# AiRyunn/BoT

Measured on NVIDIA B200. Metric: GAT layer fwd+bwd edges/sec (ogbn-proteins shape), higher is better.
Workload: dtype f32

## Files before the change

bot_b200/csrc/edge_ops.cu:

```cuda
#include "common.cuh"

namespace botgat {

static int env_pf() {
  const char* s = getenv("BOTGAT_PF");
  return (s && *s) ? atoi(s) : 0;
}

template <int PF> __device__ __forceinline__ float4 ld_rec4(const float* p) {
  float4 r;
  if constexpr (PF == 64)
    asm("ld.global.nc.L2::64B.v4.f32 {%0,%1,%2,%3}, [%4];" : "=f"(r.x), "=f"(r.y), "=f"(r.z), "=f"(r.w) : "l"(p));
  else if constexpr (PF == 128)
    asm("ld.global.nc.L2::128B.v4.f32 {%0,%1,%2,%3}, [%4];" : "=f"(r.x), "=f"(r.y), "=f"(r.z), "=f"(r.w) : "l"(p));
  else if constexpr (PF == 256)
    asm("ld.global.nc.L2::256B.v4.f32 {%0,%1,%2,%3}, [%4];" : "=f"(r.x), "=f"(r.y), "=f"(r.z), "=f"(r.w) : "l"(p));
  else
    r = __ldg(reinterpret_cast<const float4*>(p));
  return r;
}
template <int PF> __device__ __forceinline__ float2 ld_rec2(const float* p) {
  float2 r;
  if constexpr (PF == 64) asm("ld.global.nc.L2::64B.v2.f32 {%0,%1}, [%2];" : "=f"(r.x), "=f"(r.y) : "l"(p));
  else if constexpr (PF == 128) asm("ld.global.nc.L2::128B.v2.f32 {%0,%1}, [%2];" : "=f"(r.x), "=f"(r.y) : "l"(p));
  else if constexpr (PF == 256) asm("ld.global.nc.L2::256B.v2.f32 {%0,%1}, [%2];" : "=f"(r.x), "=f"(r.y) : "l"(p));
  else r = __ldg(reinterpret_cast<const float2*>(p));
  return r;
}
template <int PF> __device__ __forceinline__ float ld_rec1(const float* p) {
  float r;
  if constexpr (PF == 64) asm("ld.global.nc.L2::64B.f32 %0, [%1];" : "=f"(r) : "l"(p));
  else if constexpr (PF == 128) asm("ld.global.nc.L2::128B.f32 %0, [%1];" : "=f"(r) : "l"(p));
  else if constexpr (PF == 256) asm("ld.global.nc.L2::256B.f32 %0, [%1];" : "=f"(r) : "l"(p));
  else r = __ldg(p);
  return r;
}

constexpr int kHMax = 8;

template <int VEC, int PF> __device__ __forceinline__ void load_record(const float* rec, int H, float (&v)[kHMax]) {
  if constexpr (VEC == 4) {
#pragma unroll
    for (int q = 0; q < kHMax / 4; ++q) {
      if (q * 4 < H) {
        const float4 t = ld_rec4<PF>(rec + q * 4);
        v[q * 4] = t.x; v[q * 4 + 1] = t.y; v[q * 4 + 2] = t.z; v[q * 4 + 3] = t.w;
      }
    }
  } else if constexpr (VEC == 2) {
#pragma unroll
    for (int q = 0; q < kHMax / 2; ++q) {
      if (q * 2 < H) {
        const float2 t = ld_rec2<PF>(rec + q * 2);
        v[q * 2] = t.x; v[q * 2 + 1] = t.y;
      }
    }
  } else {
#pragma unroll
    for (int q = 0; q < kHMax; ++q)
      if (q < H) v[q] = ld_rec1<PF>(rec + q);
  }
}
template <int VEC> __device__ __forceinline__ void store_record(float* rec, int H, const float (&v)[kHMax]) {
  if constexpr (VEC == 4) {
#pragma unroll
    for (int q = 0; q < kHMax / 4; ++q)
      if (q * 4 < H) *reinterpret_cast<float4*>(rec + q * 4) = make_float4(v[q * 4], v[q * 4 + 1], v[q * 4 + 2], v[q * 4 + 3]);
  } else if constexpr (VEC == 2) {
#pragma unroll
    for (int q = 0; q < kHMax / 2; ++q)
      if (q * 2 < H) *reinterpret_cast<float2*>(rec + q * 2) = make_float2(v[q * 2], v[q * 2 + 1]);
  } else {
#pragma unroll
    for (int q = 0; q < kHMax; ++q)
      if (q < H) rec[q] = v[q];
  }
}

static int record_vec(const void* p, int64_t ld, int H) {
  auto fits = [&](int w) { return ld % w == 0 && ((uintptr_t)p % (4 * w)) == 0 && ((H + w - 1) / w) * w <= ld; };
  return fits(4) ? 4 : (fits(2) ? 2 : 1);
}

__global__ void k_pack_keep(int64_t n_edges, const uint8_t* __restrict__ keep, uint32_t* __restrict__ bits) {
  const int64_t n_round = (n_edges + 31) & ~(int64_t)31;
  for (int64_t e = blockIdx.x * (int64_t)blockDim.x + threadIdx.x; e < n_round; e += (int64_t)gridDim.x * blockDim.x) {
    const unsigned b = __ballot_sync(0xffffffffu, e < n_edges && __ldg(keep + e) != 0);
    if ((threadIdx.x & 31) == 0) bits[e >> 5] = b;
  }
}

template <int VEC, int PF>
__global__ void k_edge_stage(int64_t n_edges, int h0, int Hn, const int32_t* __restrict__ eid,
                             const int32_t* __restrict__ order,
                             const float* __restrict__ src, int64_t ld, const uint8_t* __restrict__ keep,
                             const uint32_t* __restrict__ keep_bits, float* __restrict__ dst) {
  for (int64_t t = blockIdx.x * (int64_t)blockDim.x + threadIdx.x; t < n_edges; t += (int64_t)gridDim.x * blockDim.x) {
    const int64_t p = order ? __ldg(order + t) : t;
    const int64_t e = __ldg(eid + p);
    float v[kHMax];
#pragma unroll
    for (int q = 0; q < kHMax; ++q) v[q] = 0.f;
    if (src) load_record<VEC, PF>(src + e * ld + h0, Hn, v);
    const bool dropped = keep_bits ? !((__ldg(keep_bits + (e >> 5)) >> (e & 31)) & 1u) : (keep && !__ldg(keep + e));
#pragma unroll
    for (int q = 0; q < kHMax; ++q)
      if (q < Hn) dst[(int64_t)(h0 + q) * n_edges + p] = dropped ? -INFINITY : v[q];
  }
}

template <int VEC>
__global__ void k_edge_unstage(int64_t n_edges, int h0, int Hn, int Hw, const int32_t* __restrict__ eid,
                               const int32_t* __restrict__ order,
                               const float* __restrict__ gz, float* __restrict__ dst, int64_t ld) {
  for (int64_t t = blockIdx.x * (int64_t)blockDim.x + threadIdx.x; t < n_edges; t += (int64_t)gridDim.x * blockDim.x) {
    const int64_t p = order ? __ldg(order + t) : t;
    const int64_t e = __ldg(eid + p);
    float v[kHMax];
#pragma unroll
    for (int q = 0; q < kHMax; ++q) v[q] = (q < Hn) ? __ldg(gz + (int64_t)(h0 + q) * n_edges + p) : 0.f;
    store_record<VEC>(dst + e * ld + h0, Hw, v);
  }
}

template <int VEC, int PF>
__global__ void __launch_bounds__(256)
k_edge_reduce_dst(int n_items, int H, int h0, int Hn, const int32_t* __restrict__ indptr, const int32_t* __restrict__ eid,
                  const int32_t* __restrict__ seg_row, const int32_t* __restrict__ seg_beg,
                  const int32_t* __restrict__ seg_end, const int32_t* __restrict__ seg_slot,
                  const float* __restrict__ grad_ee, int64_t ld, float* __restrict__ grad_er, float* __restrict__ scratch) {
  const int warp = threadIdx.x >> 5, lane = threadIdx.x & 31;
  const int item = blockIdx.x * 8 + warp;
  if (item >= n_items) return;
  const int v = seg_row ? seg_row[item] : item;
  const int beg = seg_row ? seg_beg[item] : indptr[v], end = seg_row ? seg_end[item] : indptr[v + 1];
  const int slot = seg_row ? seg_slot[item] : -1;
  float s[kHMax];
#pragma unroll
  for (int q = 0; q < kHMax; ++q) s[q] = 0.f;
  for (int pos = beg + lane; pos < end; pos += 32) {
    float r[kHMax];
#pragma unroll
    for (int q = 0; q < kHMax; ++q) r[q] = 0.f;
    load_record<VEC, PF>(grad_ee + (int64_t)__ldg(eid + pos) * ld + h0, Hn, r);
#pragma unroll
    for (int q = 0; q < kHMax; ++q) s[q] += r[q];
  }
#pragma unroll
  for (int q = 0; q < kHMax; ++q) {
    if (q < Hn) {
      const float t = warp_sum(s[q]);
      if (lane == 0) {
        if (slot >= 0) scratch[(int64_t)slot * H + h0 + q] = t;
        else grad_er[(int64_t)v * H + h0 + q] = t;
      }
    }
  }
}

__global__ void k_edge_reduce_combine(int n_split, int H, const int32_t* __restrict__ split_rows,
                                      const int32_t* __restrict__ split_first, const float* __restrict__ scratch,
                                      float* __restrict__ grad_er) {
  const int t = blockIdx.x * blockDim.x + threadIdx.x;
  if (t >= n_split * H) return;
  const int i = t / H, h = t - i * H;
  float a = 0.f;
  for (int s = split_first[i]; s < split_first[i + 1]; ++s) a += scratch[(int64_t)s * H + h];
  grad_er[(int64_t)split_rows[i] * H + h] = a;
}

static inline int grid_for(int64_t n, int block = 256) {
  int64_t b = (n + block - 1) / block;
  return (int)std::max<int64_t>(1, std::min<int64_t>(b, 148 * 32));
}

#define BG_PF_SWITCH(CALL)                        \
  switch (pf) {                                   \
    case 64: { constexpr int PF = 64; CALL; break; }   \
    case 128: { constexpr int PF = 128; CALL; break; } \
    case 256: { constexpr int PF = 256; CALL; break; } \
    default: { constexpr int PF = 0; CALL; break; }    \
  }

static int stage_one(const botgat_graph* g, const int32_t* eid, const int32_t* order, int H, const float* src, int64_t ld,
                     const uint8_t* keep, float* dst, cudaStream_t st) {
  const int pf = env_pf();
  uint32_t* keep_bits = nullptr;
  const bool coalesced = eid == g->in_eid && g->in_eid_identity;
  if (keep && src && g->n_edges >= (1 << 20) && !coalesced) {
    BG_CHECK(cudaMallocAsync(&keep_bits, sizeof(uint32_t) * (size_t)((g->n_edges + 31) / 32), st));
    k_pack_keep<<<grid_for(g->n_edges), 256, 0, st>>>(g->n_edges, keep, keep_bits);
    BG_LAUNCHED(1);
  }
  struct FreeBits {
    uint32_t* p; cudaStream_t st;
    ~FreeBits() { if (p) cudaFreeAsync(p, st); }
  } free_bits{keep_bits, st};
  for (int h0 = 0; h0 < H; h0 += kHMax) {
    const int Hn = std::min(kHMax, H - h0);
    const int vec = src ? record_vec(src + h0, ld, Hn) : 1;
    const int grid = order ? (int)((g->n_edges + 255) / 256) : grid_for(g->n_edges);
    if (vec == 4) { BG_PF_SWITCH((k_edge_stage<4, PF><<<grid, 256, 0, st>>>(g->n_edges, h0, Hn, eid, order, src, ld, keep, keep_bits, dst))) }
    else if (vec == 2) { BG_PF_SWITCH((k_edge_stage<2, PF><<<grid, 256, 0, st>>>(g->n_edges, h0, Hn, eid, order, src, ld, keep, keep_bits, dst))) }
    else { BG_PF_SWITCH((k_edge_stage<1, PF><<<grid, 256, 0, st>>>(g->n_edges, h0, Hn, eid, order, src, ld, keep, keep_bits, dst))) }
    BG_LAUNCHED(1);
    BG_CHECK(cudaGetLastError());
  }
  return 0;
}

}

using namespace botgat;

extern "C" int botgat_edge_stage(const botgat_graph* g, int order, int32_t H, const float* ee, int64_t ld_ee,
                                 const uint8_t* keep, const float* attn_mul, int64_t ld_am, float* eb, float* am,
                                 void* stream) {
  BG_REQUIRE(g && H > 0, "edge_stage: bad arguments");
  BG_REQUIRE(order == BOTGAT_ORDER_IN || order == BOTGAT_ORDER_OUT, "edge_stage: bad order %d", order);
  BG_REQUIRE((eb != nullptr) == (ee != nullptr || keep != nullptr), "edge_stage: eb must be given iff ee or keep is");
  BG_REQUIRE((am != nullptr) == (attn_mul != nullptr), "edge_stage: am must be given iff attn_mul is");
  BG_REQUIRE(!ee || ld_ee >= H, "edge_stage: ld_ee < H");
  BG_REQUIRE(!attn_mul || ld_am >= H, "edge_stage: ld_am < H");
  if (g->n_edges == 0 || (!eb && !am)) return 0;
  DeviceGuard guard(g->device);
  cudaStream_t st = (cudaStream_t)stream;
  const int32_t* eid = order == BOTGAT_ORDER_IN ? g->in_eid : g->out_eid;
  const int32_t* visit = order == BOTGAT_ORDER_OUT ? g->out_tile_order : nullptr;
  if (eb) {
    int rc = stage_one(g, eid, visit, ee ? H : 1, ee, ld_ee, keep, eb, st);
    if (rc) return rc;
  }
  if (am) {
    int rc = stage_one(g, eid, visit, H, attn_mul, ld_am, nullptr, am, st);
    if (rc) return rc;
  }
  return 0;
}

extern "C" int botgat_edge_unstage(const botgat_graph* g, int order, int32_t H, const float* gz, float* grad_ee,
                                   int64_t ld_gee, void* stream) {
  BG_REQUIRE(g && H > 0, "edge_unstage: bad arguments");
  BG_REQUIRE(order == BOTGAT_ORDER_IN || order == BOTGAT_ORDER_OUT, "edge_unstage: bad order %d", order);
  if (g->n_edges == 0) return 0;
  BG_REQUIRE(gz && grad_ee, "edge_unstage: null gz/grad_ee");
  BG_REQUIRE(ld_gee >= H, "edge_unstage: ld_gee < H");
  DeviceGuard guard(g->device);
  cudaStream_t st = (cudaStream_t)stream;
  const int32_t* eid = order == BOTGAT_ORDER_IN ? g->in_eid : g->out_eid;
  const int32_t* visit = order == BOTGAT_ORDER_OUT ? g->out_tile_order : nullptr;
  for (int h0 = 0; h0 < ld_gee; h0 += kHMax) {
    const int Hn = std::max(0, std::min(kHMax, H - h0));
    const int Hw = (int)std::min<int64_t>(kHMax, ld_gee - h0);
    const int vec = record_vec(grad_ee + h0, ld_gee, Hw);
    const int grid = visit ? (int)((g->n_edges + 255) / 256) : grid_for(g->n_edges);
    if (vec == 4) k_edge_unstage<4><<<grid, 256, 0, st>>>(g->n_edges, h0, Hn, Hw, eid, visit, gz, grad_ee, ld_gee);
    else if (vec == 2) k_edge_unstage<2><<<grid, 256, 0, st>>>(g->n_edges, h0, Hn, Hw, eid, visit, gz, grad_ee, ld_gee);
    else k_edge_unstage<1><<<grid, 256, 0, st>>>(g->n_edges, h0, Hn, Hw, eid, visit, gz, grad_ee, ld_gee);
    BG_LAUNCHED(1);
    BG_CHECK(cudaGetLastError());
  }
  return 0;
}

extern "C" int botgat_edge_reduce_dst(const botgat_graph* g, int32_t H, const float* grad_ee, int64_t ld_gee,
                                      float* grad_er, float* scratch, void* stream) {
  BG_REQUIRE(g && H > 0 && grad_er, "edge_reduce_dst: bad arguments");
  BG_REQUIRE(grad_ee || g->n_edges == 0, "edge_reduce_dst: null grad_ee");
  BG_REQUIRE(ld_gee >= H || g->n_edges == 0, "edge_reduce_dst: ld_gee < H");
  if (g->n_dst == 0) return 0;
  DeviceGuard guard(g->device);
  cudaStream_t st = (cudaStream_t)stream;
  const int pf = env_pf();
  const botgat_graph::SegTable& seg = g->seg_in;
  const bool split = seg.n_items > 0;
  BG_REQUIRE(!split || seg.n_slots == 0 || scratch, "edge_reduce_dst: this graph has split rows; scratch (n_slots_in*H floats) is required");
  const int n_items = split ? seg.n_items : (int)g->n_dst;
  const int32_t *sr = split ? seg.row : nullptr, *sb = seg.beg, *se = seg.end, *ss = seg.slot;
  const int grid = (n_items + 7) / 8;
  for (int h0 = 0; h0 < H; h0 += kHMax) {
    const int Hn = std::min(kHMax, H - h0);
    const int vec = g->n_edges ? record_vec(grad_ee + h0, ld_gee, Hn) : 1;
#define BG_RD(VEC) BG_PF_SWITCH((k_edge_reduce_dst<VEC, PF><<<grid, 256, 0, st>>>(n_items, H, h0, Hn, g->in_indptr, g->in_eid, sr, sb, se, ss, grad_ee, ld_gee, grad_er, scratch)))
    if (vec == 4) { BG_RD(4) } else if (vec == 2) { BG_RD(2) } else { BG_RD(1) }
#undef BG_RD
    BG_LAUNCHED(1);
    BG_CHECK(cudaGetLastError());
  }
  if (split && seg.n_split > 0) {
    const int n = seg.n_split * H;
    k_edge_reduce_combine<<<(n + 255) / 256, 256, 0, st>>>(seg.n_split, H, seg.split_rows, seg.split_first, scratch, grad_er);
    BG_LAUNCHED(1);
    BG_CHECK(cudaGetLastError());
  }
  return 0;
}
```

bot_b200/functional.py:

```python
from __future__ import annotations

import ctypes as C
import os

import torch

from . import _lib
from .graph import Graph, _stream


class KernelTimer:

    def __init__(self):
        self.events = []

    def span(self, name):
        return _Span(self, name)

    def totals(self):
        out = {}
        for name, s, e in self.events:
            n, t = out.get(name, (0, 0.0))
            out[name] = (n + 1, t + s.elapsed_time(e))
        return out


class _Span:
    def __init__(self, timer, name):
        self.timer, self.name = timer, name

    def __enter__(self):
        if self.timer is not None:
            self.s = torch.cuda.Event(enable_timing=True)
            self.s.record()

    def __exit__(self, *exc):
        if self.timer is not None:
            e = torch.cuda.Event(enable_timing=True)
            e.record()
            self.timer.events.append((self.name, self.s, e))


timer = None

edge_mode = "staged"

prestage_backward = False
_side_streams = {}


def _side_stream(device):
    key = (device.type, device.index)
    if key not in _side_streams:
        _side_streams[key] = torch.cuda.Stream(device=device)
    return _side_streams[key]


def _span(name):
    return _Span(timer, name)


def _r4(x):
    return (x + 3) // 4 * 4


def _f32c(t, name):
    if t is None:
        return None
    if t.dtype != torch.float32:
        raise TypeError(f"{name}: expected float32, got {t.dtype}")
    if not t.is_cuda:
        raise RuntimeError(f"{name}: bot_b200 has no CPU path — tensor must be on a CUDA device")
    return t.contiguous()


def _rows(t, name, H):
    if t is None:
        return None, 0
    if t.dtype != torch.float32 or not t.is_cuda:
        raise TypeError(f"{name}: expected a float32 CUDA tensor")
    if t.dim() != 2 or t.shape[1] < H:
        raise ValueError(f"{name}: expected (E, >= {H}), got {tuple(t.shape)}")
    if t.stride(1) != 1 or t.stride(0) < t.shape[1]:
        t = t.contiguous()
    return t, t.stride(0)


def pad_heads(H):
# ... 15 lines not shown
        am = torch.empty((H, E), dtype=torch.float32, device=dev)
    if eb is None and am is None:
        return None, 0, None
    ee, ld_ee = _rows(ee, "ee", H)
    attn_mul, ld_am = _rows(attn_mul, "attn_mul", H)
    with _span("edge_stage"):
        rc = _lib.load().botgat_edge_stage(graph._ensure(), order, H, _lib.ptr(ee), ld_ee, _lib.ptr(keep),
                                           _lib.ptr(attn_mul), ld_am, _lib.ptr(eb), _lib.ptr(am), _stream())
    _lib.check(rc, "botgat_edge_stage")
    return eb, Hb, am


def _check_edge_operands(graph, H, ee, keep, attn_mul):
    E = graph.number_of_edges()
    ee, ld_ee = _rows(ee, "ee", H)
    attn_mul, ld_am = _rows(attn_mul, "attn_mul", H)
    if ee is not None and ee.shape[0] != E:
        raise ValueError("ee must have one row per edge")
    if keep is not None:
        keep = keep.to(torch.uint8).contiguous()
        if keep.numel() != E:
            raise ValueError("keep must have one entry per edge")
    return ee, ld_ee, keep, attn_mul, ld_am


def _forward_core(graph, ft2d, H, D, el, er, ee, ld_ee, keep, attn_mul, ld_am, src_scale, dst_scale, slope, attn_p, seed,
                  hooks, will_backward, ep=None):
    lib = _lib.load()
    h = graph._ensure()
    dev = ft2d.device
    N_d = graph.number_of_dst_nodes()
    staged = edge_mode == "staged"
    eb_in, Hb, am_in = edge_stage(graph, _lib.ORDER_IN, H, ee, keep, attn_mul) if staged else (None, 0, None)
    pre = None
    has_edge_ops = ee is not None or keep is not None or attn_mul is not None
    if staged and prestage_backward and has_edge_ops and will_backward:
        main, side = torch.cuda.current_stream(), _side_stream(dev)
        side.wait_stream(main)
        with torch.cuda.stream(side):
            eb_o, _, am_o = edge_stage(graph, _lib.ORDER_OUT, H, ee, keep, attn_mul)
            ev = torch.cuda.Event()
            ev.record(side)
        for t in (ee, keep, attn_mul):
            if t is not None:
                t.record_stream(side)
        pre = (eb_o, am_o, ev)
    out = torch.empty((N_d, H, D), dtype=torch.float32, device=dev)
    row_max = torch.empty((N_d, H), dtype=torch.float32, device=dev)
    row_sum = torch.empty((N_d, H), dtype=torch.float32, device=dev)
    a = _lib.FwdArgs()
    a.H, a.D, a.ld_ft, a.ld_out = H, D, ft2d.stride(0), H * D
    a.ft, a.el, a.er = ft2d.data_ptr(), el.data_ptr(), (er.data_ptr() if er is not None else None)
    a.eb, a.Hb, a.col_parts = (eb_in.data_ptr() if eb_in is not None else None), Hb, 0
    a.am = am_in.data_ptr() if am_in is not None else None
    if not staged:
        if (ee is not None and ld_ee != H) or (attn_mul is not None and ld_am != H):
            raise ValueError("direct edge mode needs unpadded (E,H) edge operands")
        a.ee = ee.data_ptr() if ee is not None else None
        a.keep = keep.data_ptr() if keep is not None else None
        a.attn_mul = attn_mul.data_ptr() if attn_mul is not None else None
    a.src_scale = src_scale.data_ptr() if src_scale is not None else None
    a.dst_scale = dst_scale.data_ptr() if dst_scale is not None else None
    a.slope, a.attn_p, a.seed = float(slope), float(attn_p if attn_mul is None else 0.0), int(seed)
    a.out, a.row_max, a.row_sum = out.data_ptr(), row_max.data_ptr(), row_sum.data_ptr()
    if ep is not None:
        if will_backward:
            raise RuntimeError("the fused layer epilogue is forward-only (the backward expects the plain aggregate)")
        for key, ld in (("res", "ld_res"), ("res2", "ld_res2")):
            t = ep.get(key)
            if t is not None:
                if t.dim() != 2 or t.shape[0] < N_d or t.shape[1] < H * D or t.stride(1) != 1 or t.dtype != torch.float32:
                    raise ValueError(f"epilogue {key} must be a float32 (>= N_dst, >= H*D) matrix with unit column stride")
                setattr(a, key, t.data_ptr())
                setattr(a, ld, t.stride(0))
        if ep.get("want_y", True):
            y = torch.empty((N_d, H * D), dtype=torch.float32, device=dev)
            ep["y"] = y
            a.y, a.ld_y = y.data_ptr(), H * D
            for key, field in (("scale", "ep_scale"), ("shift", "ep_shift")):
                t = ep.get(key)
                if t is not None:
                    t = ep[key] = _f32c(t, key)
                    if t.numel() != H * D:
                        raise ValueError(f"epilogue {key} must have H*D entries")
                    setattr(a, field, t.data_ptr())
            a.ep_relu = 1 if ep.get("relu") else 0
    scratch = None
    if graph._info.n_slots_in:
        scratch = torch.empty(graph._info.n_slots_in * _r4(H * (D + 2)), dtype=torch.float32, device=dev)
        a.scratch = scratch.data_ptr()
    if hooks is not None and hooks.pre_kernel is not None:
        hooks.pre_kernel()
    chunks = hooks.head_chunks if hooks is not None and hooks.head_chunks else [(0, H)]
    for i, (hb, hc) in enumerate(chunks):
        if len(chunks) > 1 and hooks.pre_head is not None:
            hooks.pre_head(i)
        a.h_begin, a.h_count = hb, hc
        with _span("gat_fwd"):
            rc = lib.botgat_gat_forward(h, C.byref(a), _stream())
        _lib.check(rc, "botgat_gat_forward")
    return out, row_max, row_sum, pre, float(a.attn_p)


def _backward_core(graph, cfg, pre, hooks, ft2d, el, er, ee, keep, attn_mul, src_scale, dst_scale, out, row_max, row_sum,
                   gout, grad_ft2d, need_er, need_ee, hook_grad_ft=None):
    lib = _lib.load()
    h = graph._ensure()
    H, D, staged, slope, attn_p, seed = cfg
    N_s, N_d, E = ft2d.shape[0], out.shape[0], graph.number_of_edges()
    dev = ft2d.device

    def p(t):
        return t.data_ptr() if t is not None else None

    if pre is not None:
        eb_out, am_out, ev = pre
        cur = torch.cuda.current_stream()
        cur.wait_event(ev)
        for t in (eb_out, am_out):
            if t is not None:
                t.record_stream(cur)
        Hb = eb_out.shape[0] if eb_out is not None else 0
    else:
        eb_out, Hb, am_out = edge_stage(graph, _lib.ORDER_OUT, H, ee, keep, attn_mul) if staged else (None, 0, None)
    drec = torch.empty((H, N_d, 4), dtype=torch.float32, device=dev)
    gprime = torch.empty_like(gout) if dst_scale is not None else None
    grad_el = torch.empty((N_s, H), dtype=torch.float32, device=dev)
    grad_er = torch.empty((N_d, H), dtype=torch.float32, device=dev) if need_er else None
    gz = grad_ee = None
    if need_er or need_ee:
        gz = torch.empty((H, E), dtype=torch.float32, device=dev) if staged else None
        Hp = ee.shape[1] if (ee is not None and staged) else (pad_heads(H) if staged else H)
        grad_ee = torch.empty((E, Hp), dtype=torch.float32, device=dev)
    a = _lib.BwdArgs()
    a.H, a.D, a.ld_ft, a.ld_out, a.ld_gft = H, D, ft2d.stride(0), H * D, grad_ft2d.stride(0)
    a.ft, a.el, a.er = ft2d.data_ptr(), el.data_ptr(), p(er)
    a.eb_out, a.Hb, a.phases, a.am_out = p(eb_out), Hb, 0, p(am_out)
    if not staged:
        a.ee, a.keep, a.attn_mul = p(ee), p(keep), p(attn_mul)
    a.src_scale, a.dst_scale = p(src_scale), p(dst_scale)
    a.slope, a.attn_p, a.seed = slope, attn_p, seed
    a.out, a.row_max, a.row_sum, a.gout = out.data_ptr(), row_max.data_ptr(), row_sum.data_ptr(), gout.data_ptr()
    a.drec, a.gprime, a.gz = drec.data_ptr(), p(gprime), p(gz)
    scratch = None
    if graph._info.n_slots_out or graph._info.n_slots_in:
        scratch = torch.empty(graph._info.n_slots_out * _r4(H * (D + 1)) + graph._info.n_slots_in * H,
                              dtype=torch.float32, device=dev)
        a.scratch = scratch.data_ptr()
    a.grad_ft, a.grad_el, a.grad_ee, a.grad_er = grad_ft2d.data_ptr(), grad_el.data_ptr(), p(grad_ee), p(grad_er)
    a.ld_gee = grad_ee.stride(0) if grad_ee is not None else 0
    post_src = hooks.post_src if hooks is not None else None
    chunks = hooks.head_chunks if hooks is not None and hooks.head_chunks else None
    if chunks is not None and (len(chunks) > 1 or getattr(hooks, "force_chunked", False)):
        a.phases = 1
        _lib.check(lib.botgat_gat_backward(h, C.byref(a), _stream()), "botgat_gat_backward")
        for i, (hb, hc) in enumerate(chunks):
            a.phases, a.h_begin, a.h_count = 2, hb, hc
# ... 25 lines not shown
    return grad_el, grad_er, (grad_ee if need_ee else None)


BWD_MAX_D = 1024


class GATFusedFn(torch.autograd.Function):

    @staticmethod
    def forward(ctx, graph, ft, el, er, ee, keep, attn_mul, src_scale, dst_scale, slope, attn_p, seed, hooks=None):
        if ft.dim() != 3:
            raise ValueError("ft must be (N_src, H, D)")
        ft = _f32c(ft, "ft")
        N_s, H, D = ft.shape
        N_d = graph.number_of_dst_nodes()
        if N_s != graph.number_of_src_nodes():
            raise ValueError(f"ft has {N_s} rows, graph has {graph.number_of_src_nodes()} source nodes")
        el = _f32c(el, "el").view(N_s, H)
        er = None if er is None else _f32c(er, "er").view(N_d, H)
        ee, ld_ee, keep, attn_mul, ld_am = _check_edge_operands(graph, H, ee, keep, attn_mul)
        src_scale, dst_scale = _f32c(src_scale, "src_scale"), _f32c(dst_scale, "dst_scale")
        Dk = D
        if any(ctx.needs_input_grad):
            if D > BWD_MAX_D:
                raise ValueError(f"GAT layer with gradients: head width D={D} exceeds the backward's limit of {BWD_MAX_D} "
                                 "columns per head (inference without gradients has no such limit)")
            vw = 4 if D % 4 == 0 and ft.data_ptr() % 16 == 0 else 2 if D % 2 == 0 and ft.data_ptr() % 8 == 0 else 1
            if D > 256 * vw:
                if hooks is not None:
                    raise ValueError(f"GAT layer with hooks: D={D} > {256 * vw} needs a multiple of 4 and a 16-byte aligned ft")
                Dk = _r4(D)
                ft = torch.cat([ft, ft.new_zeros(N_s, H, Dk - D)], 2)
        with torch.cuda.device(ft.device):
            out, row_max, row_sum, pre, attn_p_used = _forward_core(
                graph, ft.view(N_s, H * Dk), H, Dk, el, er, ee, ld_ee, keep, attn_mul, ld_am, src_scale, dst_scale, slope,
                attn_p, seed, hooks, any(ctx.needs_input_grad))
        ctx.graph = graph
        ctx.hooks = hooks
        ctx.pre = pre
        ctx.D = D
        ctx.cfg = (H, Dk, edge_mode == "staged", float(slope), attn_p_used, int(seed))
        ctx.save_for_backward(ft, el, er, ee, keep, attn_mul, src_scale, dst_scale, out, row_max, row_sum)
        return out if Dk == D else out[:, :, :D].contiguous()

    @staticmethod
    def backward(ctx, gout):
        ft, el, er, ee, keep, attn_mul, src_scale, dst_scale, out, row_max, row_sum = ctx.saved_tensors
        H, D = ctx.cfg[0], ctx.cfg[1]
        need_er = er is not None and ctx.needs_input_grad[3]
        need_ee = ee is not None and ctx.needs_input_grad[4]
        gout = _f32c(gout, "grad_out")
        if D != ctx.D:
            gout = torch.cat([gout, gout.new_zeros(gout.shape[0], H, D - ctx.D)], 2)
        elif D > 256 and gout.data_ptr() % 16:
            gout = gout.clone()
        grad_ft = torch.empty_like(ft)
        with torch.cuda.device(ft.device):
            grad_el, grad_er, grad_ee = _backward_core(
                ctx.graph, ctx.cfg, ctx.pre, ctx.hooks, ft.view(-1, H * D), el, er, ee, keep, attn_mul, src_scale, dst_scale,
                out, row_max, row_sum, gout, grad_ft.view(-1, H * D), need_er, need_ee, hook_grad_ft=grad_ft)
        if D != ctx.D:
            grad_ft = grad_ft[:, :, :ctx.D]
        return (None, grad_ft, grad_el, grad_er, grad_ee, None, None, None, None, None, None, None, None)


def _pad_rows(w, rows):
    if w.shape[0] == rows:
        return w
    return torch.cat([w, w.new_zeros(rows - w.shape[0], w.shape[1])], 0)


class GATConvSampledFn(torch.autograd.Function):

    @staticmethod
    def forward(ctx, graph, x_src, x_dst, w_src, w_dst, b_dst, ee, keep, attn_mul, dst_scale, H, D, slope, attn_p, seed,
                src_scale=None):
        x_src, x_dst = _f32c(x_src, "feat_src"), _f32c(x_dst, "feat_dst")
        N_s, N_d, HD = graph.number_of_src_nodes(), graph.number_of_dst_nodes(), H * D
        if x_src.shape[0] != N_s or x_dst.shape[0] != N_d:
            raise ValueError("feat_src / feat_dst rows do not match the graph")
        has_er = w_dst.shape[0] == HD + H
        P = (HD + H + 31) // 32 * 32
        ws, wd = _pad_rows(w_src, P), _pad_rows(w_dst, P)
        bd = torch.cat([b_dst, b_dst.new_zeros(P - HD)])
        ee, ld_ee, keep, attn_mul, ld_am = _check_edge_operands(graph, H, ee, keep, attn_mul)
        dst_scale, src_scale = _f32c(dst_scale, "dst_scale"), _f32c(src_scale, "src_scale")
        vw = 4 if D % 4 == 0 else 2 if D % 2 == 0 else 1
        if any(ctx.needs_input_grad) and D > min(256 * vw, BWD_MAX_D):
            raise ValueError(f"GAT layer with gradients: head width D={D} exceeds the backward's limit of {256 * vw} columns "
                             f"per head at {vw}-float vectors (at most {BWD_MAX_D}, for D a multiple of 4)")
        with torch.cuda.device(x_src.device):
            Ys = x_src @ ws.t()
            Yd = torch.addmm(bd, x_dst, wd.t())
            el = Ys[:, HD:HD + H].contiguous() if src_scale is None else Ys[:, HD:HD + H] * src_scale.unsqueeze(-1)
            er = Yd[:, HD:HD + H].contiguous() if has_er else None
            out, row_max, row_sum, pre, attn_p_used = _forward_core(
                graph, Ys, H, D, el, er, ee, ld_ee, keep, attn_mul, ld_am, src_scale, dst_scale, slope, attn_p, seed, None,
                any(ctx.needs_input_grad))
            rst = out + Yd[:, :HD].view(N_d, H, D)
        ctx.graph, ctx.pre, ctx.same_x = graph, pre, x_dst is x_src or x_dst.data_ptr() == x_src.data_ptr() and N_s == N_d
        ctx.cfg = (H, D, edge_mode == "staged", float(slope), attn_p_used, int(seed))
        ctx.dims = (P, has_er, w_src.shape[0], w_dst.shape[0])
        ctx.save_for_backward(x_src, x_dst, ws, wd, Ys, el, er, ee, keep, attn_mul, dst_scale, out, row_max, row_sum, src_scale)
        return rst

    @staticmethod
    def backward(ctx, grst):
        x_src, x_dst, ws, wd, Ys, el, er, ee, keep, attn_mul, dst_scale, out, row_max, row_sum, src_scale = ctx.saved_tensors
        H, D = ctx.cfg[0], ctx.cfg[1]
        P, has_er, rows_s, rows_d = ctx.dims
        HD = H * D
        need = ctx.needs_input_grad
        need_ee = ee is not None and need[6]
        grst = _f32c(grst, "grad_out")
        N_s, N_d = x_src.shape[0], x_dst.shape[0]
        dev = x_src.device
        with torch.cuda.device(dev):
            gYs = torch.empty((N_s, P), dtype=torch.float32, device=dev)
            gYd = torch.empty((N_d, P), dtype=torch.float32, device=dev)
            grad_el, grad_er, grad_ee = _backward_core(
                ctx.graph, ctx.cfg, ctx.pre, None, Ys, el, er, ee, keep, attn_mul, src_scale, dst_scale, out, row_max, row_sum,
                grst, gYs, has_er, need_ee)
            gYs[:, HD:HD + H] = grad_el if src_scale is None else grad_el * src_scale.unsqueeze(-1)
            gYs[:, HD + H:].zero_()
            gYd[:, :HD] = grst.view(N_d, HD)
            if has_er:
                gYd[:, HD:HD + H] = grad_er
                gYd[:, HD + H:].zero_()
            else:
                gYd[:, HD:].zero_()
            gw_s = (gYs.t() @ x_src)[:rows_s] if need[3] else None
            gw_d = (gYd.t() @ x_dst)[:rows_d] if need[4] else None
            gb = grst.view(N_d, HD).sum(0) if need[5] else None
            gx_s = gx_d = None
            if ctx.same_x and need[1]:
                gx_s = torch.addmm(gYs @ ws, gYd, wd)
            else:
                gx_s = gYs @ ws if need[1] else None
                gx_d = gYd @ wd if need[2] else None
        return (None, gx_s, gx_d, gw_s, gw_d, gb, grad_ee, None, None, None, None, None, None, None, None, None)


class LayerTail:

    def __init__(self, h_last=None, norm=None, relu=False):
        self.h_last, self.norm, self.relu = h_last, norm, relu

    def usable(self):
        if os.environ.get("BOTGAT_FUSE_TAIL", "1") == "0":
            return False
        n = self.norm
        if isinstance(n, torch.nn.BatchNorm1d):
            return not n.training and n.running_mean is not None
        return n is None or (hasattr(n, "weight") and hasattr(n, "bias"))

    def scale_shift(self):
        n = self.norm
        if n is None:
            return None, None
        if isinstance(n, torch.nn.BatchNorm1d):
            scale = torch.rsqrt(n.running_var + n.eps)
            if n.weight is not None:
                scale = scale * n.weight
            shift = -n.running_mean * scale
            if n.bias is not None:
                shift = shift + n.bias
            return scale.detach(), shift.detach()
        return (None if n.weight is None else n.weight.detach()), (None if n.bias is None else n.bias.detach())


def gat_fused_inference(graph, ft, el, er, ee, keep, attn_mul, src_scale, dst_scale, slope, tail, res=None):
    with torch.no_grad():
        ft = _f32c(ft, "ft")
        N_s, H, D = ft.shape
        N_d = graph.number_of_dst_nodes()
        el = _f32c(el, "el").view(N_s, H)
        er = None if er is None else _f32c(er, "er").view(N_d, H)
        ee, ld_ee, keep, attn_mul, ld_am = _check_edge_operands(graph, H, ee, keep, attn_mul)
        src_scale, dst_scale = _f32c(src_scale, "src_scale"), _f32c(dst_scale, "dst_scale")
        scale, shift = tail.scale_shift()
        h_last = tail.h_last
        if h_last is not None:
            h_last = _f32c(h_last, "h_last").view(h_last.shape[0], -1)
        if res is not None:
            res = _f32c(res, "res").view(res.shape[0], -1)
        ep = {"res": res, "res2": h_last, "scale": scale, "shift": shift, "relu": tail.relu, "want_y": True}
        with torch.cuda.device(ft.device):
            out, _, _, _, _ = _forward_core(graph, ft.view(N_s, H * D), H, D, el, er, ee, ld_ee, keep, attn_mul, ld_am, src_scale,
                                            dst_scale, slope, 0.0, 0, None, False, ep=ep)
        return out.view(N_d, H * D), ep["y"]


def gat_conv_inference(graph, x_src, x_dst, w_src, w_dst, b_dst, ee, keep, attn_mul, dst_scale, H, D, slope, tail,
                       src_scale=None):
    with torch.no_grad():
        x_src, x_dst = _f32c(x_src, "feat_src"), _f32c(x_dst, "feat_dst")
        N_s, N_d, HD = graph.number_of_src_nodes(), graph.number_of_dst_nodes(), H * D
        if x_src.shape[0] != N_s or x_dst.shape[0] != N_d:
            raise ValueError("feat_src / feat_dst rows do not match the graph")
        has_er = w_dst.shape[0] == HD + H
        P = (HD + H + 31) // 32 * 32
        ws, wd = _pad_rows(w_src, P), _pad_rows(w_dst, P)
        bd = torch.cat([b_dst, b_dst.new_zeros(P - HD)])
        ee, ld_ee, keep, attn_mul, ld_am = _check_edge_operands(graph, H, ee, keep, attn_mul)
        dst_scale, src_scale = _f32c(dst_scale, "dst_scale"), _f32c(src_scale, "src_scale")
        scale, shift = tail.scale_shift()
        h_last = tail.h_last
        if h_last is not None:
            h_last = _f32c(h_last, "h_last").view(h_last.shape[0], -1)
        ep = {"res2": h_last, "scale": scale, "shift": shift, "relu": tail.relu, "want_y": True}
        with torch.cuda.device(x_src.device):
            Ys = x_src @ ws.t()
            Yd = torch.addmm(bd, x_dst, wd.t())
            ep["res"] = Yd
            el = Ys[:, HD:HD + H].contiguous() if src_scale is None else Ys[:, HD:HD + H] * src_scale.unsqueeze(-1)
            er = Yd[:, HD:HD + H].contiguous() if has_er else None
            out, _, _, _, _ = _forward_core(graph, Ys, H, D, el, er, ee, ld_ee, keep, attn_mul, ld_am, src_scale, dst_scale,
                                            slope, 0.0, 0, None, False, ep=ep)
        return out.view(N_d, HD), ep["y"]


class EdgeLogitProj(torch.autograd.Function):

    @staticmethod
    def forward(ctx, x, weight):
        lib = _lib.load()
        x = _f32c(x, "feat_edge")
        weight = _f32c(weight, "weight")
        E, Cin = x.shape
        H = weight.shape[0]
        y = torch.empty((E, pad_heads(H)), dtype=torch.float32, device=x.device)
        with torch.cuda.device(x.device):
            with _span("edge_proj_fwd"):
                rc = lib.botgat_edge_proj_forward(E, Cin, H, x.data_ptr(), x.stride(0), weight.data_ptr(), y.data_ptr(),
                                                  y.stride(0), x.device.index, _stream())
        _lib.check(rc, "botgat_edge_proj_forward")
        ctx.save_for_backward(x, weight)
        return y

    @staticmethod
    def backward(ctx, gy):
        lib = _lib.load()
        x, weight = ctx.saved_tensors
        E, Cin = x.shape
        H = weight.shape[0]
        gy, ld_gy = _rows(gy, "grad_ee", H)
        gx = torch.empty_like(x) if ctx.needs_input_grad[0] else None
        gw = torch.empty_like(weight) if ctx.needs_input_grad[1] else None
        partials = torch.empty(lib.botgat_edge_proj_gw_blocks() * H * Cin, dtype=torch.float32, device=x.device) \
            if gw is not None else None
# ... 144 lines not shown
```

bot_b200/partition.py:

```python
from __future__ import annotations

import os

import torch
import torch.distributed as dist

from .graph import Graph


def partition_bounds(dst, n_nodes, n_parts):
    counts = torch.bincount(dst, minlength=n_nodes)
    indptr = torch.zeros(n_nodes + 1, dtype=torch.int64, device=dst.device)
    indptr[1:] = torch.cumsum(counts, 0)
    e = int(dst.numel())
    targets = torch.tensor([(p * e) // n_parts for p in range(1, n_parts)], dtype=torch.int64, device=dst.device)
    inner = torch.searchsorted(indptr, targets, right=False).clamp(max=n_nodes)
    bounds = torch.cat([torch.zeros(1, dtype=torch.int64, device=dst.device), inner,
                        torch.full((1,), n_nodes, dtype=torch.int64, device=dst.device)])
    return torch.cummax(bounds, 0).values


class _DenseHalo(torch.autograd.Function):

    @staticmethod
# ... 149 lines not shown
        n_own = pg.n_own
        graph = pg.local
        main = torch.cuda.current_stream()
        if hx.fwd_pending:
            hx.h_table.barrier(channel=0)
        hx.fwd_pending, hx.bwd_pending = True, False
        if ft_own.data_ptr() != hx.own_ft.data_ptr():
            hx.own[:, :HD].copy_(ft_own.reshape(n_own, HD))
        if el_own.data_ptr() != hx.own_el.data_ptr():
            hx.own_el.copy_(el_own.reshape(n_own, H))
        hx.h_table.barrier(channel=1)
        hx.stream.wait_stream(main)
        events = []
        with torch.cuda.stream(hx.stream):
            for i, (hb, hc) in enumerate(chunks):
                if i == 0:
                    hx.pull(HD, H)
                hx.pull(hb * D, hc * D)
                ev = torch.cuda.Event()
                ev.record(hx.stream)
                events.append(ev)
        el_all = torch.empty((hx.table.shape[0], H), dtype=torch.float32, device=hx.table.device)

        def pre_kernel():
            main.wait_event(events[0])
            el_all.copy_(hx.table[:, HD:HD + H])

        def pre_head(i):
            if i > 0:
                main.wait_event(events[i])

        ee, ld_ee, keep, attn_mul, ld_am = Fn._check_edge_operands(graph, H, ee, keep, attn_mul)
        hooks = Fn.Hooks(pre_kernel=pre_kernel, head_chunks=chunks, pre_head=pre_head)
        out, row_max, row_sum, pre, attn_p_used = Fn._forward_core(
            graph, hx.table, H, D, el_all, er, ee, ld_ee, keep, attn_mul, ld_am, src_scale, dst_scale, slope, attn_p, seed,
            hooks, True)
        ctx.pg, ctx.hx, ctx.chunks = pg, hx, chunks
        ctx.cfg = (H, D, Fn.edge_mode == "staged", float(slope), attn_p_used, int(seed))
        ctx.save_for_backward(el_all, er, ee, keep, attn_mul, src_scale, dst_scale, out, row_max, row_sum)
        return out

    @staticmethod
    def backward(ctx, gout):
        from . import functional as Fn

        pg, hx, chunks = ctx.pg, ctx.hx, ctx.chunks
        el_all, er, ee, keep, attn_mul, src_scale, dst_scale, out, row_max, row_sum = ctx.saved_tensors
        H, D, HD = hx.H, hx.D, hx.HD
        n_own = pg.n_own
        main = torch.cuda.current_stream()
        gout = gout.contiguous()
        gshard = torch.empty((hx.rows, hx.P), dtype=torch.float32, device=gout.device)
        gshard.record_stream(hx.stream)
        if hx.bwd_pending or not hx.fwd_pending:
            hx.h_gtable.barrier(channel=0)
        hx.bwd_pending, hx.fwd_pending = True, False

        def post_src_head(i, grad_ft, grad_el):
            hb, hc = chunks[i]
            last = i == len(chunks) - 1
            if last:
                hx.gtable[:, HD:HD + H].copy_(grad_el)
            ev = torch.cuda.Event()
            ev.record(main)
            with torch.cuda.stream(hx.stream):
                hx.stream.wait_event(ev)
                hx.h_gtable.barrier(channel=1 + i)
                hx.pull_reduce(hb * D, hc * D, gshard)
                if last:
                    hx.pull_reduce(HD, H, gshard)

        hooks = Fn.Hooks(head_chunks=chunks, post_src_head=post_src_head)
        hooks.force_chunked = True
        need_er = er is not None and ctx.needs_input_grad[5]
        need_ee = ee is not None and ctx.needs_input_grad[6]
        grad_el, grad_er, grad_ee = Fn._backward_core(
            pg.local, ctx.cfg, None, hooks, hx.table, el_all, er, ee, keep, attn_mul, src_scale, dst_scale, out, row_max, row_sum,
            gout, hx.gtable, need_er, need_ee)
        main.wait_stream(hx.stream)
        grad_ft_own = gshard[:n_own, :HD].unflatten(1, (H, D))
        grad_el_own = gshard[:n_own, HD:HD + H]
        return (None, None, None, grad_ft_own, grad_el_own, grad_er, grad_ee, None, None, None, None, None, None, None)


class PartitionedGraph:

    def __init__(self, src, dst, n_nodes, world=None, rank=None, group=None, plan="auto", build_graph=True):
        self.group = group
        self.pipeline_heads = os.environ.get("BOTGAT_PIPE_HEADS", "0") == "1"
        self.exchange = os.environ.get("BOTGAT_EXCHANGE", "auto")
        self.halo_chunks = int(os.environ.get("BOTGAT_HALO_CHUNKS", "0"))
        self._p2p, self._p2p_failed, self._p2p_error = {}, False, None
        self.world = dist.get_world_size(group) if world is None else world
        self.rank = dist.get_rank(group) if rank is None else rank
        self.n_nodes = n_nodes
        dev = src.device
        self.bounds = partition_bounds(dst, n_nodes, self.world)
        b = self.bounds.tolist()
        self.lo, self.hi = b[self.rank], b[self.rank + 1]
        self.n_own = self.hi - self.lo
        self.max_own = max(b[i + 1] - b[i] for i in range(self.world))

        mine = torch.nonzero((dst >= self.lo) & (dst < self.hi)).flatten()
        self.edge_gid = mine
        s, d = src.index_select(0, mine), dst.index_select(0, mine)
        ldst = d - self.lo
        owned = (s >= self.lo) & (s < self.hi)
        self.halo_gid = torch.unique(s[~owned])
        if plan == "auto":
            plan = "dense" if (self.halo_gid.numel() + self.n_own) * 2 >= n_nodes else "sparse"
# ... 186 lines not shown
```

Baseline: 2.765 billion.

## Add 256-bit v8 record loads/stores, one-thread-per-edge staging, skip identity eid

Adds Blackwell 256-bit vector global loads and stores (ld/st .v8.f32) for edge records with stride divisible by 8, so a full 8-head record moves in one instruction. The stage and unstage kernels change from grid-stride loops to one thread per edge, with launch bounds and 32-bit indices. When the edge-id permutation is the identity, the eid gather is skipped. The unused prestage-backward side-stream path is removed from the Python code. The v8 path depends on PTX support for 256-bit accesses and on 32-byte alignment checks.

```diff
diff --git a/bot_b200/csrc/edge_ops.cu b/bot_b200/csrc/edge_ops.cu
--- a/bot_b200/csrc/edge_ops.cu
+++ b/bot_b200/csrc/edge_ops.cu
@@ -36,10 +36,21 @@
   return r;
 }
 
+#define BG_V8_OUT "=f"(v[0]), "=f"(v[1]), "=f"(v[2]), "=f"(v[3]), "=f"(v[4]), "=f"(v[5]), "=f"(v[6]), "=f"(v[7])
+template <int PF> __device__ __forceinline__ void ld_rec8(const float* p, float (&v)[8]) {
+  if constexpr (PF == 64) asm("ld.global.nc.L2::64B.v8.f32 {%0,%1,%2,%3,%4,%5,%6,%7}, [%8];" : BG_V8_OUT : "l"(p));
+  else if constexpr (PF == 128) asm("ld.global.nc.L2::128B.v8.f32 {%0,%1,%2,%3,%4,%5,%6,%7}, [%8];" : BG_V8_OUT : "l"(p));
+  else if constexpr (PF == 256) asm("ld.global.nc.L2::256B.v8.f32 {%0,%1,%2,%3,%4,%5,%6,%7}, [%8];" : BG_V8_OUT : "l"(p));
+  else asm("ld.global.nc.v8.f32 {%0,%1,%2,%3,%4,%5,%6,%7}, [%8];" : BG_V8_OUT : "l"(p));
+}
+#undef BG_V8_OUT
+
 constexpr int kHMax = 8;
 
 template <int VEC, int PF> __device__ __forceinline__ void load_record(const float* rec, int H, float (&v)[kHMax]) {
-  if constexpr (VEC == 4) {
+  if constexpr (VEC == 8) {
+    ld_rec8<PF>(rec, v);
+  } else if constexpr (VEC == 4) {
 #pragma unroll
     for (int q = 0; q < kHMax / 4; ++q) {
       if (q * 4 < H) {
@@ -62,7 +73,10 @@
   }
 }
 template <int VEC> __device__ __forceinline__ void store_record(float* rec, int H, const float (&v)[kHMax]) {
-  if constexpr (VEC == 4) {
+  if constexpr (VEC == 8) {
+    asm volatile("st.global.v8.f32 [%0], {%1,%2,%3,%4,%5,%6,%7,%8};" ::"l"(rec), "f"(v[0]), "f"(v[1]), "f"(v[2]), "f"(v[3]),
+                 "f"(v[4]), "f"(v[5]), "f"(v[6]), "f"(v[7]) : "memory");
+  } else if constexpr (VEC == 4) {
 #pragma unroll
     for (int q = 0; q < kHMax / 4; ++q)
       if (q * 4 < H) *reinterpret_cast<float4*>(rec + q * 4) = make_float4(v[q * 4], v[q * 4 + 1], v[q * 4 + 2], v[q * 4 + 3]);
@@ -79,7 +93,7 @@
 
 static int record_vec(const void* p, int64_t ld, int H) {
   auto fits = [&](int w) { return ld % w == 0 && ((uintptr_t)p % (4 * w)) == 0 && ((H + w - 1) / w) * w <= ld; };
-  return fits(4) ? 4 : (fits(2) ? 2 : 1);
+  return fits(8) ? 8 : fits(4) ? 4 : (fits(2) ? 2 : 1);
 }
 
 __global__ void k_pack_keep(int64_t n_edges, const uint8_t* __restrict__ keep, uint32_t* __restrict__ bits) {
@@ -90,38 +104,42 @@
   }
 }
 
+constexpr int kStageBlock = 256, kStageMinBlocks = 8;
+
 template <int VEC, int PF>
-__global__ void k_edge_stage(int64_t n_edges, int h0, int Hn, const int32_t* __restrict__ eid,
-                             const int32_t* __restrict__ order,
-                             const float* __restrict__ src, int64_t ld, const uint8_t* __restrict__ keep,
-                             const uint32_t* __restrict__ keep_bits, float* __restrict__ dst) {
-  for (int64_t t = blockIdx.x * (int64_t)blockDim.x + threadIdx.x; t < n_edges; t += (int64_t)gridDim.x * blockDim.x) {
-    const int64_t p = order ? __ldg(order + t) : t;
-    const int64_t e = __ldg(eid + p);
-    float v[kHMax];
-#pragma unroll
-    for (int q = 0; q < kHMax; ++q) v[q] = 0.f;
-    if (src) load_record<VEC, PF>(src + e * ld + h0, Hn, v);
-    const bool dropped = keep_bits ? !((__ldg(keep_bits + (e >> 5)) >> (e & 31)) & 1u) : (keep && !__ldg(keep + e));
-#pragma unroll
-    for (int q = 0; q < kHMax; ++q)
-      if (q < Hn) dst[(int64_t)(h0 + q) * n_edges + p] = dropped ? -INFINITY : v[q];
-  }
+__global__ void __launch_bounds__(kStageBlock, kStageMinBlocks)
+k_edge_stage(int64_t n_edges, int h0, int Hn, const int32_t* __restrict__ eid, const int32_t* __restrict__ order,
+             const float* __restrict__ src, int64_t ld, const uint8_t* __restrict__ keep,
+             const uint32_t* __restrict__ keep_bits, float* __restrict__ dst) {
+  const int64_t t = (int64_t)blockIdx.x * kStageBlock + threadIdx.x;
+  if (t >= n_edges) return;
+  const int p = order ? __ldg(order + t) : (int)t;
+  const int e = eid ? __ldg(eid + p) : p;
+  float v[kHMax];
+#pragma unroll
+  for (int q = 0; q < kHMax; ++q) v[q] = 0.f;
+  if (src) load_record<VEC, PF>(src + (int64_t)e * ld + h0, Hn, v);
+  const bool dropped = keep_bits ? !((__ldg(keep_bits + (e >> 5)) >> (e & 31)) & 1u) : (keep && !__ldg(keep + e));
+#pragma unroll
+  for (int q = 0; q < kHMax; ++q)
+    if (q < Hn) dst[(int64_t)(h0 + q) * n_edges + p] = dropped ? -INFINITY : v[q];
 }
 
 template <int VEC>
-__global__ void k_edge_unstage(int64_t n_edges, int h0, int Hn, int Hw, const int32_t* __restrict__ eid,
-                               const int32_t* __restrict__ order,
-                               const float* __restrict__ gz, float* __restrict__ dst, int64_t ld) {
-  for (int64_t t = blockIdx.x * (int64_t)blockDim.x + threadIdx.x; t < n_edges; t += (int64_t)gridDim.x * blockDim.x) {
-    const int64_t p = order ? __ldg(order + t) : t;
-    const int64_t e = __ldg(eid + p);
-    float v[kHMax];
-#pragma unroll
-    for (int q = 0; q < kHMax; ++q) v[q] = (q < Hn) ? __ldg(gz + (int64_t)(h0 + q) * n_edges + p) : 0.f;
-    store_record<VEC>(dst + e * ld + h0, Hw, v);
-  }
-}
+__global__ void __launch_bounds__(kStageBlock, kStageMinBlocks)
+k_edge_unstage(int64_t n_edges, int h0, int Hn, int Hw, const int32_t* __restrict__ eid,
+               const int32_t* __restrict__ order, const float* __restrict__ gz, float* __restrict__ dst, int64_t ld) {
+  const int64_t t = (int64_t)blockIdx.x * kStageBlock + threadIdx.x;
+  if (t >= n_edges) return;
+  const int p = order ? __ldg(order + t) : (int)t;
+  const int e = __ldg(eid + p);
+  float v[kHMax];
+#pragma unroll
+  for (int q = 0; q < kHMax; ++q) v[q] = (q < Hn) ? __ldg(gz + (int64_t)(h0 + q) * n_edges + p) : 0.f;
+  store_record<VEC>(dst + (int64_t)e * ld + h0, Hw, v);
+}
+
+static inline int grid_for_stage(int64_t n) { return (int)((n + kStageBlock - 1) / kStageBlock); }
 
 template <int VEC, int PF>
 __global__ void __launch_bounds__(256)
@@ -142,7 +160,7 @@
     float r[kHMax];
 #pragma unroll
     for (int q = 0; q < kHMax; ++q) r[q] = 0.f;
-    load_record<VEC, PF>(grad_ee + (int64_t)__ldg(eid + pos) * ld + h0, Hn, r);
+    load_record<VEC, PF>(grad_ee + (int64_t)(eid ? __ldg(eid + pos) : pos) * ld + h0, Hn, r);
 #pragma unroll
     for (int q = 0; q < kHMax; ++q) s[q] += r[q];
   }
@@ -187,6 +205,7 @@
   const int pf = env_pf();
   uint32_t* keep_bits = nullptr;
   const bool coalesced = eid == g->in_eid && g->in_eid_identity;
+  if (coalesced) eid = nullptr;
   if (keep && src && g->n_edges >= (1 << 20) && !coalesced) {
     BG_CHECK(cudaMallocAsync(&keep_bits, sizeof(uint32_t) * (size_t)((g->n_edges + 31) / 32), st));
     k_pack_keep<<<grid_for(g->n_edges), 256, 0, st>>>(g->n_edges, keep, keep_bits);
@@ -199,10 +218,10 @@
   for (int h0 = 0; h0 < H; h0 += kHMax) {
     const int Hn = std::min(kHMax, H - h0);
     const int vec = src ? record_vec(src + h0, ld, Hn) : 1;
-    const int grid = order ? (int)((g->n_edges + 255) / 256) : grid_for(g->n_edges);
-    if (vec == 4) { BG_PF_SWITCH((k_edge_stage<4, PF><<<grid, 256, 0, st>>>(g->n_edges, h0, Hn, eid, order, src, ld, keep, keep_bits, dst))) }
-    else if (vec == 2) { BG_PF_SWITCH((k_edge_stage<2, PF><<<grid, 256, 0, st>>>(g->n_edges, h0, Hn, eid, order, src, ld, keep, keep_bits, dst))) }
-    else { BG_PF_SWITCH((k_edge_stage<1, PF><<<grid, 256, 0, st>>>(g->n_edges, h0, Hn, eid, order, src, ld, keep, keep_bits, dst))) }
+    const int grid = grid_for_stage(g->n_edges);
+#define BG_ST(VEC) BG_PF_SWITCH((k_edge_stage<VEC, PF><<<grid, kStageBlock, 0, st>>>(g->n_edges, h0, Hn, eid, order, src, ld, keep, keep_bits, dst)))
+    if (vec == 8) { BG_ST(8) } else if (vec == 4) { BG_ST(4) } else if (vec == 2) { BG_ST(2) } else { BG_ST(1) }
+#undef BG_ST
     BG_LAUNCHED(1);
     BG_CHECK(cudaGetLastError());
   }
@@ -253,10 +272,11 @@
     const int Hn = std::max(0, std::min(kHMax, H - h0));
     const int Hw = (int)std::min<int64_t>(kHMax, ld_gee - h0);
     const int vec = record_vec(grad_ee + h0, ld_gee, Hw);
-    const int grid = visit ? (int)((g->n_edges + 255) / 256) : grid_for(g->n_edges);
-    if (vec == 4) k_edge_unstage<4><<<grid, 256, 0, st>>>(g->n_edges, h0, Hn, Hw, eid, visit, gz, grad_ee, ld_gee);
-    else if (vec == 2) k_edge_unstage<2><<<grid, 256, 0, st>>>(g->n_edges, h0, Hn, Hw, eid, visit, gz, grad_ee, ld_gee);
-    else k_edge_unstage<1><<<grid, 256, 0, st>>>(g->n_edges, h0, Hn, Hw, eid, visit, gz, grad_ee, ld_gee);
+    const int grid = grid_for_stage(g->n_edges);
+    if (vec == 8) k_edge_unstage<8><<<grid, kStageBlock, 0, st>>>(g->n_edges, h0, Hn, Hw, eid, visit, gz, grad_ee, ld_gee);
+    else if (vec == 4) k_edge_unstage<4><<<grid, kStageBlock, 0, st>>>(g->n_edges, h0, Hn, Hw, eid, visit, gz, grad_ee, ld_gee);
+    else if (vec == 2) k_edge_unstage<2><<<grid, kStageBlock, 0, st>>>(g->n_edges, h0, Hn, Hw, eid, visit, gz, grad_ee, ld_gee);
+    else k_edge_unstage<1><<<grid, kStageBlock, 0, st>>>(g->n_edges, h0, Hn, Hw, eid, visit, gz, grad_ee, ld_gee);
     BG_LAUNCHED(1);
     BG_CHECK(cudaGetLastError());
   }
@@ -278,11 +298,12 @@
   const int n_items = split ? seg.n_items : (int)g->n_dst;
   const int32_t *sr = split ? seg.row : nullptr, *sb = seg.beg, *se = seg.end, *ss = seg.slot;
   const int grid = (n_items + 7) / 8;
+  const int32_t* in_eid = g->in_eid_identity ? nullptr : g->in_eid;
   for (int h0 = 0; h0 < H; h0 += kHMax) {
     const int Hn = std::min(kHMax, H - h0);
     const int vec = g->n_edges ? record_vec(grad_ee + h0, ld_gee, Hn) : 1;
-#define BG_RD(VEC) BG_PF_SWITCH((k_edge_reduce_dst<VEC, PF><<<grid, 256, 0, st>>>(n_items, H, h0, Hn, g->in_indptr, g->in_eid, sr, sb, se, ss, grad_ee, ld_gee, grad_er, scratch)))
-    if (vec == 4) { BG_RD(4) } else if (vec == 2) { BG_RD(2) } else { BG_RD(1) }
+#define BG_RD(VEC) BG_PF_SWITCH((k_edge_reduce_dst<VEC, PF><<<grid, 256, 0, st>>>(n_items, H, h0, Hn, g->in_indptr, in_eid, sr, sb, se, ss, grad_ee, ld_gee, grad_er, scratch)))
+    if (vec == 8) { BG_RD(8) } else if (vec == 4) { BG_RD(4) } else if (vec == 2) { BG_RD(2) } else { BG_RD(1) }
 #undef BG_RD
     BG_LAUNCHED(1);
     BG_CHECK(cudaGetLastError());
diff --git a/bot_b200/functional.py b/bot_b200/functional.py
--- a/bot_b200/functional.py
+++ b/bot_b200/functional.py
@@ -44,16 +44,6 @@
 timer = None
 
 edge_mode = "staged"
-
-prestage_backward = False
-_side_streams = {}
-
-
-def _side_stream(device):
-    key = (device.type, device.index)
-    if key not in _side_streams:
-        _side_streams[key] = torch.cuda.Stream(device=device)
-    return _side_streams[key]
 
 
 def _span(name):
@@ -135,19 +125,6 @@
     N_d = graph.number_of_dst_nodes()
     staged = edge_mode == "staged"
     eb_in, Hb, am_in = edge_stage(graph, _lib.ORDER_IN, H, ee, keep, attn_mul) if staged else (None, 0, None)
-    pre = None
-    has_edge_ops = ee is not None or keep is not None or attn_mul is not None
-    if staged and prestage_backward and has_edge_ops and will_backward:
-        main, side = torch.cuda.current_stream(), _side_stream(dev)
-        side.wait_stream(main)
-        with torch.cuda.stream(side):
-            eb_o, _, am_o = edge_stage(graph, _lib.ORDER_OUT, H, ee, keep, attn_mul)
-            ev = torch.cuda.Event()
-            ev.record(side)
-        for t in (ee, keep, attn_mul):
-            if t is not None:
-                t.record_stream(side)
-        pre = (eb_o, am_o, ev)
     out = torch.empty((N_d, H, D), dtype=torch.float32, device=dev)
     row_max = torch.empty((N_d, H), dtype=torch.float32, device=dev)
     row_sum = torch.empty((N_d, H), dtype=torch.float32, device=dev)
@@ -202,10 +179,10 @@
         with _span("gat_fwd"):
             rc = lib.botgat_gat_forward(h, C.byref(a), _stream())
         _lib.check(rc, "botgat_gat_forward")
-    return out, row_max, row_sum, pre, float(a.attn_p)
-
-
-def _backward_core(graph, cfg, pre, hooks, ft2d, el, er, ee, keep, attn_mul, src_scale, dst_scale, out, row_max, row_sum,
+    return out, row_max, row_sum, float(a.attn_p)
+
+
+def _backward_core(graph, cfg, hooks, ft2d, el, er, ee, keep, attn_mul, src_scale, dst_scale, out, row_max, row_sum,
                    gout, grad_ft2d, need_er, need_ee, hook_grad_ft=None):
     lib = _lib.load()
     h = graph._ensure()
@@ -216,16 +193,7 @@
     def p(t):
         return t.data_ptr() if t is not None else None
 
-    if pre is not None:
-        eb_out, am_out, ev = pre
-        cur = torch.cuda.current_stream()
-        cur.wait_event(ev)
-        for t in (eb_out, am_out):
-            if t is not None:
-                t.record_stream(cur)
-        Hb = eb_out.shape[0] if eb_out is not None else 0
-    else:
-        eb_out, Hb, am_out = edge_stage(graph, _lib.ORDER_OUT, H, ee, keep, attn_mul) if staged else (None, 0, None)
+    eb_out, Hb, am_out = edge_stage(graph, _lib.ORDER_OUT, H, ee, keep, attn_mul) if staged else (None, 0, None)
     drec = torch.empty((H, N_d, 4), dtype=torch.float32, device=dev)
     gprime = torch.empty_like(gout) if dst_scale is not None else None
     grad_el = torch.empty((N_s, H), dtype=torch.float32, device=dev)
@@ -317,12 +285,11 @@
                 Dk = _r4(D)
                 ft = torch.cat([ft, ft.new_zeros(N_s, H, Dk - D)], 2)
         with torch.cuda.device(ft.device):
-            out, row_max, row_sum, pre, attn_p_used = _forward_core(
+            out, row_max, row_sum, attn_p_used = _forward_core(
                 graph, ft.view(N_s, H * Dk), H, Dk, el, er, ee, ld_ee, keep, attn_mul, ld_am, src_scale, dst_scale, slope,
                 attn_p, seed, hooks, any(ctx.needs_input_grad))
         ctx.graph = graph
         ctx.hooks = hooks
-        ctx.pre = pre
         ctx.D = D
         ctx.cfg = (H, Dk, edge_mode == "staged", float(slope), attn_p_used, int(seed))
         ctx.save_for_backward(ft, el, er, ee, keep, attn_mul, src_scale, dst_scale, out, row_max, row_sum)
@@ -342,7 +309,7 @@
         grad_ft = torch.empty_like(ft)
         with torch.cuda.device(ft.device):
             grad_el, grad_er, grad_ee = _backward_core(
-                ctx.graph, ctx.cfg, ctx.pre, ctx.hooks, ft.view(-1, H * D), el, er, ee, keep, attn_mul, src_scale, dst_scale,
+                ctx.graph, ctx.cfg, ctx.hooks, ft.view(-1, H * D), el, er, ee, keep, attn_mul, src_scale, dst_scale,
                 out, row_max, row_sum, gout, grad_ft.view(-1, H * D), need_er, need_ee, hook_grad_ft=grad_ft)
         if D != ctx.D:
             grad_ft = grad_ft[:, :, :ctx.D]
@@ -379,11 +346,11 @@
             Yd = torch.addmm(bd, x_dst, wd.t())
             el = Ys[:, HD:HD + H].contiguous() if src_scale is None else Ys[:, HD:HD + H] * src_scale.unsqueeze(-1)
             er = Yd[:, HD:HD + H].contiguous() if has_er else None
-            out, row_max, row_sum, pre, attn_p_used = _forward_core(
+            out, row_max, row_sum, attn_p_used = _forward_core(
                 graph, Ys, H, D, el, er, ee, ld_ee, keep, attn_mul, ld_am, src_scale, dst_scale, slope, attn_p, seed, None,
                 any(ctx.needs_input_grad))
             rst = out + Yd[:, :HD].view(N_d, H, D)
-        ctx.graph, ctx.pre, ctx.same_x = graph, pre, x_dst is x_src or x_dst.data_ptr() == x_src.data_ptr() and N_s == N_d
+        ctx.graph, ctx.same_x = graph, x_dst is x_src or x_dst.data_ptr() == x_src.data_ptr() and N_s == N_d
         ctx.cfg = (H, D, edge_mode == "staged", float(slope), attn_p_used, int(seed))
         ctx.dims = (P, has_er, w_src.shape[0], w_dst.shape[0])
         ctx.save_for_backward(x_src, x_dst, ws, wd, Ys, el, er, ee, keep, attn_mul, dst_scale, out, row_max, row_sum, src_scale)
@@ -404,7 +371,7 @@
             gYs = torch.empty((N_s, P), dtype=torch.float32, device=dev)
             gYd = torch.empty((N_d, P), dtype=torch.float32, device=dev)
             grad_el, grad_er, grad_ee = _backward_core(
-                ctx.graph, ctx.cfg, ctx.pre, None, Ys, el, er, ee, keep, attn_mul, src_scale, dst_scale, out, row_max, row_sum,
+                ctx.graph, ctx.cfg, None, Ys, el, er, ee, keep, attn_mul, src_scale, dst_scale, out, row_max, row_sum,
                 grst, gYs, has_er, need_ee)
             gYs[:, HD:HD + H] = grad_el if src_scale is None else grad_el * src_scale.unsqueeze(-1)
             gYs[:, HD + H:].zero_()
@@ -471,7 +438,7 @@
             res = _f32c(res, "res").view(res.shape[0], -1)
         ep = {"res": res, "res2": h_last, "scale": scale, "shift": shift, "relu": tail.relu, "want_y": True}
         with torch.cuda.device(ft.device):
-            out, _, _, _, _ = _forward_core(graph, ft.view(N_s, H * D), H, D, el, er, ee, ld_ee, keep, attn_mul, ld_am, src_scale,
+            out, _, _, _ = _forward_core(graph, ft.view(N_s, H * D), H, D, el, er, ee, ld_ee, keep, attn_mul, ld_am, src_scale,
                                             dst_scale, slope, 0.0, 0, None, False, ep=ep)
         return out.view(N_d, H * D), ep["y"]
 
@@ -500,7 +467,7 @@
             ep["res"] = Yd
             el = Ys[:, HD:HD + H].contiguous() if src_scale is None else Ys[:, HD:HD + H] * src_scale.unsqueeze(-1)
             er = Yd[:, HD:HD + H].contiguous() if has_er else None
-            out, _, _, _, _ = _forward_core(graph, Ys, H, D, el, er, ee, ld_ee, keep, attn_mul, ld_am, src_scale, dst_scale,
+            out, _, _, _ = _forward_core(graph, Ys, H, D, el, er, ee, ld_ee, keep, attn_mul, ld_am, src_scale, dst_scale,
                                             slope, 0.0, 0, None, False, ep=ep)
         return out.view(N_d, HD), ep["y"]
 
diff --git a/bot_b200/partition.py b/bot_b200/partition.py
--- a/bot_b200/partition.py
+++ b/bot_b200/partition.py
@@ -205,7 +205,7 @@
 
         ee, ld_ee, keep, attn_mul, ld_am = Fn._check_edge_operands(graph, H, ee, keep, attn_mul)
         hooks = Fn.Hooks(pre_kernel=pre_kernel, head_chunks=chunks, pre_head=pre_head)
-        out, row_max, row_sum, pre, attn_p_used = Fn._forward_core(
+        out, row_max, row_sum, attn_p_used = Fn._forward_core(
             graph, hx.table, H, D, el_all, er, ee, ld_ee, keep, attn_mul, ld_am, src_scale, dst_scale, slope, attn_p, seed,
             hooks, True)
         ctx.pg, ctx.hx, ctx.chunks = pg, hx, chunks
@@ -248,7 +248,7 @@
         need_er = er is not None and ctx.needs_input_grad[5]
         need_ee = ee is not None and ctx.needs_input_grad[6]
         grad_el, grad_er, grad_ee = Fn._backward_core(
-            pg.local, ctx.cfg, None, hooks, hx.table, el_all, er, ee, keep, attn_mul, src_scale, dst_scale, out, row_max, row_sum,
+            pg.local, ctx.cfg, hooks, hx.table, el_all, er, ee, keep, attn_mul, src_scale, dst_scale, out, row_max, row_sum,
             gout, hx.gtable, need_er, need_ee)
         main.wait_stream(hx.stream)
         grad_ft_own = gshard[:n_own, :HD].unflatten(1, (H, D))
```

Result: faster. 2.833 billion, median of 6 (+2.4%).
